# TMZZ22331/Robust-Speech-Emotion-Recognition-via-Dynamic-Asymmetric-Distillation-in-Noisy-Environments

Hardware: AMD Instinct MI355X
Metric: utterances/sec (DAD train step) batch=64 at 1/2/4/8 MI355X; loss parity (higher is better)
Workload: dtype fp16

## Files before the change

### robust-speech-emotion-recognition-via-dynamic-asymmetric-distillation-in-noisy-environments_amd/csrc/dad_abi.hip

```cpp
#include <string.h>

#include "dad_host.h"
#include "dad_timing.h"

constexpr int kMaxDevices = 64;

int device_cus(int* out) {
  static int cache[kMaxDevices];
  int dev = 0;
  DAD_TRY(hipGetDevice(&dev));
  if (dev < 0 || dev >= kMaxDevices) return DAD_E_ARG;
  if (!cache[dev]) DAD_TRY(hipDeviceGetAttribute(&cache[dev], hipDeviceAttributeMultiprocessorCount, dev));
  *out = cache[dev];
  return DAD_OK;
}

namespace {

inline DadStoreRows store_rows_of(const dad_batch* bt) { return DadStoreRows{bt->rowc, bt->lenc, bt->rown, bt->lenn}; }

DadPrepArgs prep_args(const dad_config* cfg, const dad_batch* bt, uint16_t* x16) {
  DadPrepArgs p;
  memset(&p, 0, sizeof(p));
  const Keys k = keys_of(cfg);
// ... 111 lines not shown
  memset(&pa, 0, sizeof(pa));
  pa.g = s.G; pa.warmup = cfg->warmup;
  pa.mc = bt->mc; pa.mn = bt->mn; pa.part_sum = s.ws.part_sum;
  pa.student = s.st->student; pa.teacher = s.st->teacher;
  if (s.explicit_rng()) { pa.keep1 = bt->keep1; pa.keep2 = bt->keep2; }
  pa.key_drop1 = s.k.drop1; pa.key_drop2 = s.k.drop2;
  pa.p_drop = cfg->p_drop; pa.drop_scale = cfg->drop_scale;
  pa.emb = s.st->emb; pa.vlen = s.ws.vlen; pa.logits = s.st->logits;
  pa.part_cnt = s.ws.part_cnt; pa.cnt_tot = s.ws.cnt_tot;
  pa.eflag = s.ws.eflag; pa.tail_terms = s.st->tail + DAD_T_ECDA_TERM;
  pa.range_flag = reinterpret_cast<uint32_t*>(s.st->tail + DAD_T_RANGE);
  if (cfg->ragged) { pa.lenc = bt->lenc; pa.lenn = bt->lenn; }
  if (!s.plan.pool_grid) pa.ready = s.ws.pool_ready;
  return pa;
}

DadTailArgs tail_args(const Step& s) {
  DadTailArgs ta;
  memset(&ta, 0, sizeof(ta));
  ta.cfg = *s.cfg; ta.yc = s.bt->yc; ta.logits = s.st->logits; ta.emb = s.st->emb; ta.student = s.st->student;
  if (s.explicit_rng()) { ta.keep1 = s.bt->keep1; ta.keep2 = s.bt->keep2; }
  ta.key_drop1 = s.k.drop1; ta.key_drop2 = s.k.drop2;
  ta.dacp = s.st->dacp; ta.tailf = s.st->tail; ta.ge = s.ws.ge; ta.ge_ecda = s.ws.ge_ecda; ta.grad = s.st->grad;
  ta.gzb = s.ws.gzb; ta.eflag = s.ws.eflag;
  return ta;
}

DadEcdaArgs ecda_args(const Step& s) {
  DadEcdaArgs ca;
  memset(&ca, 0, sizeof(ca));
  ca.cfg = *s.cfg; ca.yc = s.bt->yc; ca.emb = s.st->emb; ca.tailf = s.st->tail;
  ca.tail_terms = s.st->tail + DAD_T_ECDA_TERM; ca.ge = s.ws.ge_ecda; ca.scratch = s.ws.ecda; ca.eflag = s.ws.eflag;
  ca.sink = s.ws.gflat;
  return ca;
}

DadWgradArgs wgrad_args(const Step& s) {
  const dad_config* cfg = s.cfg;
  const dad_batch* bt = s.bt;
  DadWgradArgs wa;
  memset(&wa, 0, sizeof(wa));
  wa.g = s.G; wa.warmup = cfg->warmup;
  wa.mask_len = cfg->mask_len; wa.start_hi = cfg->start_hi;
  wa.xc = static_cast<const float*>(bt->xc); wa.xn = static_cast<const float*>(bt->xn);
  wa.src = store_rows_of(bt);
  if (s.explicit_rng()) { wa.ns = bt->ns; wa.u = bt->u; wa.start = bt->start; }
  wa.key_strong = s.k.strong; wa.key_feat = s.k.feat; wa.key_tstart = s.k.tstart;
  wa.strong_std = cfg->strong_std; wa.feat_p = cfg->feat_p;
  wa.bits = s.ws.bits; wa.ge = s.ws.ge; wa.vlen = s.ws.vlen; wa.xs16 = s.ws.set_of(cfg);
  wa.splits = s.plan.splits; wa.ntiles = s.plan.wgrad_tiles;
  wa.wpart = s.ws.wpart;
  return wa;
}

DadReduceArgs reduce_args(const Step& s) {
  const dad_config* cfg = s.cfg;
  DadReduceArgs ra;
  memset(&ra, 0, sizeof(ra));
  ra.g = s.G; ra.warmup = cfg->warmup;
  ra.want_norm = cfg->dp_world == 1;
  ra.w_kl = cfg->w_kl; ra.w_ecda = cfg->w_ecda;
  ra.w_scl = s.plan.scl_n ? cfg->w_scl : 0.0f;
  ra.ge_ecda = s.ws.ge_ecda;
  ra.gzb = s.ws.gzb; ra.eflag = s.ws.eflag; ra.student = s.st->student; ra.emb = s.st->emb;
  if (s.explicit_rng()) { ra.keep1 = s.bt->keep1; ra.keep2 = s.bt->keep2; }
  ra.key_drop1 = s.k.drop1; ra.key_drop2 = s.k.drop2; ra.p_drop = cfg->p_drop; ra.drop_scale = cfg->drop_scale;
// ... 314 lines not shown
```

### robust-speech-emotion-recognition-via-dynamic-asymmetric-distillation-in-noisy-environments_amd/csrc/dad_kernels.h

```cpp
#pragma once
#include "dad_common.h"

#define DAD_ENC_F32_THREADS 256
#define DAD_ENC_WS_THREADS 512
#define DAD_ENC_WS_MAXJ 256
#define DAD_POOL_THREADS 64
#define DAD_TAIL_THREADS 512
#define DAD_ECDA_THREADS 512
#define DAD_WGRAD_THREADS 256
#define WGD_DB 64
#define WGD_NDB (DAD_D / WGD_DB)
#define WGD_MAXU 64
#ifndef WGD_DEPTH
#define WGD_DEPTH 4
#endif
#define WGD_XP 96
#ifndef WGD_GROUPS
#define WGD_GROUPS 2
#endif
#define WGD_THREADS (256 * WGD_GROUPS)
#define WGD_XWG 4
#define DAD_REDUCE_THREADS 256
#define DAD_REDUCE_COLS 256
#define DAD_REDUCE_XBLK 16
// ... 54 lines not shown
  float weak_std, strong_std, feat_p;
  uint16_t* x16;
  __host__ __device__ int xc_type() const { return src_types & 0xff; }
  __host__ __device__ int xn_type() const { return (src_types >> 8) & 0xff; }
};


struct DadTailArgs {
  dad_config cfg;
  const int64_t* yc;
  const float* logits; const float* emb;
  const float* student;
  const uint8_t* keep1; const uint8_t* keep2;
  uint32_t key_drop1, key_drop2;
  float* dacp;
  float* tailf;
  float* ge;
  float* ge_ecda;
  float* gzb;
  uint32_t* eflag;
  float* grad;
};

struct DadEcdaArgs {
  dad_config cfg;
  const int64_t* yc;
  const float* emb;
  const float* tailf;
  float* tail_terms;
  float* ge;
  uint32_t* eflag;
  float* scratch;
  float* sink;
};

struct DadWgradArgs {
  DadGeom g;
  int warmup, splits, mask_len, start_hi;
  const float* xc; const float* xn;
  DadStoreRows src;
  const float* ns; const float* u; const int64_t* start;
  uint32_t key_strong, key_feat, key_tstart;
  float strong_std, feat_p;
  const uint32_t* bits; const float* ge; const float* vlen;
  const uint16_t* xs16;
  float* wpart;
  int ntiles;
};

struct DadReduceArgs {
  DadGeom g;
  int splits, warmup, want_norm;
  float w_kl, w_ecda;
  const float* wpart; const float* ge; const float* vlen; const float* cnt_tot;
  const float* ge_ecda;
  const float* gzb; const uint32_t* eflag;
  const float* student; const float* emb;
  const uint8_t* keep1; const uint8_t* keep2;
  uint32_t key_drop1, key_drop2;
  float p_drop, drop_scale;
  const float* tailf;
  float* grad; float* normpart;
  const uint32_t* pool_abort;
  float w_scl;
};

// ... 69 lines not shown
```

### robust-speech-emotion-recognition-via-dynamic-asymmetric-distillation-in-noisy-environments_amd/csrc/step_plan.h

```cpp
#pragma once
#include <stdlib.h>
#include <string.h>

#include <algorithm>
#include <vector>

#include "dad_kernels.h"
#include "scl.h"

inline int check_cfg(const dad_config* c) {
  if (!c) return DAD_E_ARG;
  if (c->B < 1 || c->B > DAD_MAX_BATCH || c->T < 1) return DAD_E_SHAPE;
  if (c->Bn < 0 || c->Bn > DAD_MAX_BATCH || c->Tn < 0) return DAD_E_SHAPE;
  if (!c->warmup && (c->Bn < 1 || c->Tn < 1)) return DAD_E_SHAPE;
  if (c->precision != DAD_PREC_FP32 && !dad_prec16(c->precision)) return DAD_E_ARG;
  if (c->rng_mode != DAD_RNG_EXPLICIT && c->rng_mode != DAD_RNG_COUNTER) return DAD_E_ARG;
  if (c->dp_world < 1) return DAD_E_ARG;
  if (c->ragged && !dad_prec16(c->precision)) return DAD_E_UNSUPPORTED;
  if (c->scl_on && !(scl_tau_ok(c->scl_tau) && c->w_scl >= -3.402823466e38f && c->w_scl <= 3.402823466e38f)) return DAD_E_ARG;
  return DAD_OK;
}

inline bool scl_in_step(const dad_config* c) { return c->scl_on && !c->warmup; }

// ... 5 lines not shown
inline bool store_dtype_ok(int t) { return t == DAD_STORE_F32 || t == DAD_STORE_F16 || t == DAD_STORE_BF16; }
inline int check_batch_dtypes(const dad_config* c, const dad_batch* b) {
  if (!store_dtype_ok(b->xc_dtype) || !store_dtype_ok(b->xn_dtype)) return DAD_E_ARG;
  if ((!b->rowc && b->xc_dtype != DAD_STORE_F32) || (!b->rown && b->xn_dtype != DAD_STORE_F32)) return DAD_E_ARG;
  if ((b->xc_dtype != DAD_STORE_F32 || b->xn_dtype != DAD_STORE_F32) && !dad_prec16(c->precision))
    return DAD_E_UNSUPPORTED;
  return DAD_OK;
}
inline int check_ragged_batch(const dad_config* c, const dad_batch* b) {
  if (!c->ragged) return DAD_OK;
  if (!b->rowc || !b->lenc) return DAD_E_ARG;
  if ((b->xn || !c->warmup) && (!b->rown || !b->lenn)) return DAD_E_ARG;
  return DAD_OK;
}
inline bool has_explicit_draws(const dad_batch* b) { return b->nw && b->ns && b->u && b->start; }

inline int splits_of(const dad_config* c) {
  const DadGeom g = geom_of(c);
  if (c->splits <= 0) return dad_auto_splits(g, c->precision, c->warmup);
  if (!dad_prec16(c->precision)) return c->splits;
  return std::max(c->splits, dad_wgd_min_splits(dad_wg_total(g, c->warmup)));
}

inline int max_splits_of(const dad_config* c) {
  const int s = splits_of(c);
  if (!c->warmup) return s;
  dad_config post = *c;
  post.warmup = 0;
  return std::max(s, splits_of(&post));
}

inline bool tail_w_on() {
  static const bool on = [] { const char* e = getenv("DAD_TAIL_W"); return !(e && strcmp(e, "0") == 0); }();
  return on;
}

inline int wp_max_range(const DadGeom& G, int Bn, int nt, int ns) {
  int worst = 0;
  for (int wg = 0; wg < nt + ns; ++wg) {
    bool t = false;
    int j0 = 0, j1 = 0;
    dad_wp_job_range(wg, nt, ns, G.Bc, G.Tc, G.ncc, Bn, G.Tn, G.ncn, Bn * G.ncn, t, j0, j1);
    worst = std::max(worst, j1 - j0);
  }
  return worst;
}
inline int wp_split(const DadGeom& G, int Bn, int cus, int& nt, int& ns) {
  struct Entry { int Bc, Tc, Bn, Tn, cus, rc, nt, ns; };
  static thread_local Entry last{-1, -1, -1, -1, -1, 0, 0, 0};
  if (!(last.Bc == G.Bc && last.Tc == G.Tc && last.Bn == Bn && last.Tn == G.Tn && last.cus == cus)) {
    Entry e{G.Bc, G.Tc, Bn, G.Tn, cus, 0, 0, 0};
    const int Js = Bn * G.ncn, Jc = G.Bc * G.ncc;
    const double ln = (double)Bn * ((G.Tn + 15) / 16), lc = (double)G.Bc * ((G.Tc + 15) / 16);
    if (Js == 0) {
      e.ns = std::min(cus, Jc);
    } else {
      e.nt = std::max(1, std::min(std::min(Js, cus - 1), (int)(cus * ln / (2.0 * ln + lc) + 0.5)));
      e.ns = std::min(cus - e.nt, Jc + Js);
    }
    while (e.rc == DAD_OK && wp_max_range(G, Bn, e.nt, e.ns) > DAD_ENC_WS_MAXJ) {
      if (e.nt > 0 && e.nt < Js) ++e.nt;
      if (e.ns < Jc + Js) ++e.ns;
      if (e.nt + e.ns > Js + Jc + 2) e.rc = DAD_E_SHAPE;
    }
    last = e;
  }
// ... 204 lines not shown
```

### robust-speech-emotion-recognition-via-dynamic-asymmetric-distillation-in-noisy-environments_amd/csrc/tail_w.hip

```cpp
#include "dad_prep.h"
#include "dad_probe.h"
#include "pool.h"
#include "tail_common.h"

#define ECDA_SLOTS 32
DAD_PROBE_BUFFER(ecda_stamps, DAD_C * ECDA_SLOTS + 16)
DAD_PROBE_BUFFER(prep_stamps, 256 * 8 * 2)
#define ECDA_STAMP(k) \
  if (threadIdx.x == 0) DAD_PROBE_SET(ecda_stamps, (blockIdx.x - 1) * ECDA_SLOTS + (k), DAD_PROBE_WALL())
#define ECDA_CYC(k)                                                                          \
  do {                                                                                       \
    __builtin_amdgcn_sched_barrier(0);                                                       \
    if (threadIdx.x == 0) DAD_PROBE_SET(ecda_stamps, (blockIdx.x - 1) * ECDA_SLOTS + (k), DAD_PROBE_CLK()); \
    __builtin_amdgcn_sched_barrier(0);                                                       \
  } while (0)
#define ECDA_STAMP_SIZES(c, n, ns) \
  do { DAD_PROBE_SET(ecda_stamps, (c) * ECDA_SLOTS + 10, (n)); DAD_PROBE_SET(ecda_stamps, (c) * ECDA_SLOTS + 11, (ns)); } while (0)
#define TAIL_STAMP(k) \
  if (threadIdx.x == 0) DAD_PROBE_SET(ecda_stamps, DAD_C * ECDA_SLOTS + (k), DAD_PROBE_WALL())
#define TAIL_CYCLES(k) \
  if (threadIdx.x == 0) DAD_PROBE_SET(ecda_stamps, DAD_C * ECDA_SLOTS + (k), DAD_PROBE_CLK())

#define TAIL_STAMP_W1(k) \
  if (threadIdx.x == 64 && blockIdx.x == 0) DAD_PROBE_SET(ecda_stamps, DAD_C * ECDA_SLOTS + (k), DAD_PROBE_WALL())

#define TW_MAXB 64
#define EW_ZP 260
#define EW_CP 68
#define EW_CPW 132
#define EW_GP 33

struct DacpBlockScratch {
  int rk[ECDA_THREADS / 64][TW_MAXB];
  float srt[ECDA_THREADS / 64][DAD_C][TW_MAXB];
};

struct DacpState {
  float tau[DAD_C], Q[DAD_C], anc[DAD_C];
};

template <int N>
__device__ __forceinline__ float dpp_seg_sum(float v) {
  static_assert(N == 4 || N == 8 || N == 16 || N == 32, "segment");
  v += dad_dpp_f<0x111>(v);
  v += dad_dpp_f<0x112>(v);
  if constexpr (N >= 8) v += dad_dpp_f<0x114>(v);
  if constexpr (N >= 16) v += dad_dpp_f<0x118>(v);
  if constexpr (N == 32) v += dad_dpp_f<0x142, 0xa>(v);
  return v;
}
__device__ __forceinline__ DacpState dacp_state_of(float dv) {
  DacpState d;
#pragma unroll
  for (int k = 0; k < DAD_C; ++k) {
    d.tau[k] = __int_as_float(__builtin_amdgcn_readlane(__float_as_int(dv), k));
    d.Q[k] = __int_as_float(__builtin_amdgcn_readlane(__float_as_int(dv), 4 + k));
    d.anc[k] = __int_as_float(__builtin_amdgcn_readlane(__float_as_int(dv), 16 + k));
  }
  return d;
}

__device__ __forceinline__ void dacp_block8(const dad_config& cfg, int Bn, float s, int p, const DacpState& D,
                                            DacpBlockScratch& W, float (&tau)[DAD_C], float (&wc)[DAD_C],
// ... 190 lines not shown
struct __attribute__((aligned(16))) EcdaW {
  union {
    float zc[(TW_MAXB + 1) * EW_ZP];
    float dbw[2 * TW_MAXB * EW_CPW];
  } a;
  union {
    DacpBlockScratch dw;
    float gp[10][32 * EW_GP];
  } b;
  union {
    float cp[ECDA_THREADS / 64][DAD_C][DAD_H];
    float dbn[TW_MAXB * EW_CP];
  } c;
  float cent[DAD_C][DAD_H];
  float nz[2 * TW_MAXB], wz[2 * TW_MAXB], rs[2 * TW_MAXB];
  int rowz[2 * TW_MAXB], mem[2 * TW_MAXB];
  int cnt[DAD_C];
  float pd[DAD_C][DAD_C];
  float msp[ECDA_THREADS / 64][DAD_H];
  double nsp[ECDA_THREADS / 64];
  double t3p[ECDA_THREADS / 64][3];
  float cmp[ECDA_THREADS / 64];
};

__device__ __forceinline__ int ew_pair(int ti, int tj, int nt) { return ti * nt - ti * (ti - 1) / 2 + (tj - ti); }
__device__ __forceinline__ void ew_pair_inv(int pr, int nt, int& ti, int& tj) {
  ti = 0;
  while (pr >= nt - ti) { pr -= nt - ti; ++ti; }
  tj = ti + pr;
}

#define EW_TP 40
static_assert(ECDA_NG * 32 * EW_TP <= sizeof(EcdaW::b) / sizeof(float), "ew_member_grads: a 32 x EW_TP tile per wave in S.b");
__device__ __forceinline__ int ew_nk64(int ncand_all) { return max((ncand_all + 7) >> 3, 5); }

template <int NP, int NK, class RG>
__device__ __forceinline__ void ew_member_grads(EcdaW& S, const float* db, int dp, int c, int ncs, int ncand_all,
                                                float mmd_scale, float comp_scale, float* ge_c, float* ge_s,
                                                float* sink, const RG& repg_at) {
  static_assert(NK >= 1 && NK <= NP / 8, "ew_member_grads: NK 8-candidate blocks of NP");
  const int tid = threadIdx.x, lane = tid & 63;
  const int g = __builtin_amdgcn_readfirstlane(tid >> 6);
  const int kh = lane >> 5, l32 = lane & 31;
  for (int item = g; item < (NP / 32) * (DAD_H / 32); item += ECDA_NG) {
    const int ti = item >> 3, tc = item & 7;
    const int d = 32 * tc + l32;
    const float* ra = &db[(32 * ti + l32) * dp + 4 * kh];
    f32x4 av[NK];
    float bv[NK][4];
#pragma unroll
    for (int q = 0; q < NK; ++q) {
      av[q] = *reinterpret_cast<const f32x4*>(ra + 8 * q);
#pragma unroll
      for (int e = 0; e < 4; ++e) bv[q][e] = S.a.zc[(8 * q + 4 * kh + e) * EW_ZP + d];
    }
    float zi[16], rsv[16];
#pragma unroll
    for (int r = 0; r < 16; ++r) {
      const int i = 32 * ti + dad_acc_row(r, kh);
      const int ic = i < ncand_all ? i : 0;
      zi[r] = S.a.zc[i * EW_ZP + d];
      rsv[r] = S.rs[ic];
    }
    const float mu = S.cent[c][d], rg = repg_at(d);
    f32x16 acc = f32x16{};
#pragma unroll
    for (int q = 0; q < NK; ++q)
#pragma unroll
      for (int e = 0; e < 4; ++e) acc = __builtin_amdgcn_mfma_f32_32x32x2f32(av[q][e], bv[q][e], acc, 0, 0, 0);
    ECDA_CYC(25);
    float* stg = &S.b.gp[0][0] + g * (32 * EW_TP);
#pragma unroll
    for (int r = 0; r < 16; ++r) {
      const int i = 32 * ti + dad_acc_row(r, kh);
      const bool noisy = i >= ncs;
      stg[dad_acc_row(r, kh) * EW_TP + l32] =
          mmd_scale * (2.0f * (rsv[r] * zi[r] - acc[r])) + (noisy ? comp_scale * (zi[r] - mu) + rg : 0.0f);
    }
    asm volatile("s_waitcnt lgkmcnt(0)" ::: "memory");
    ECDA_CYC(26);
    const int rl = lane >> 3, c4 = 4 * (lane & 7);
#pragma unroll
    for (int k = 0; k < 4; ++k) {
      const int row = rl + 8 * k, i = 32 * ti + row;
      const int ic = i < ncand_all ? i : 0;
      const bool mem = (i < ncand_all) & (S.mem[ic] != 0);
      const f32x4 v = *reinterpret_cast<const f32x4*>(stg + row * EW_TP + c4);
      float* dst = mem ? (i >= ncs ? ge_s : ge_c) + (size_t)S.rowz[ic] * DAD_H + 32 * tc + c4 : sink + 32 * tc + c4;
      *reinterpret_cast<f32x4*>(dst) = v;
    }
    asm volatile("s_waitcnt lgkmcnt(0)" ::: "memory");
    ECDA_CYC(27);
  }
}

template <bool WIDE>
__device__ __forceinline__ void ecda_class_w(const DadEcdaArgs& a, const int c, EcdaW& S, const WaveMask& M,
                                             const f32x4 (&ps)[ECDA_PRE_U], const int prd,
                                             const int ncls, const int nvalid, const int npairs, const bool gc,
                                             const bool rep_on, const float rep_coef, const float att_c, const int ncs,
                                             const int ncand_all, const double wsum_t) {
  const dad_config& cfg = a.cfg;
  const int B = cfg.B, Bn = cfg.Bn;
  const int tid = threadIdx.x, lane = tid & 63;
  const int g = __builtin_amdgcn_readfirstlane(tid >> 6);
  const int kh = lane >> 5, l32 = lane & 31;
  const float* emb_c = a.emb;
  const float* emb_s = a.emb + (size_t)(B + Bn) * DAD_H;
  const int npad = ncand_all <= 32 ? 32 : (ncand_all <= 64 ? 64 : 128);
  const int nt = npad / 32;
  const int npt = nt * (nt + 1) / 2;
  const int ks = npt == 1 ? 8 : (npt == 3 ? 2 : 1);
  float* db = WIDE ? S.a.dbw : S.c.dbn;
  const int dp = WIDE ? EW_CPW : EW_CP;
  const int cnc = S.cnt[c];
  const int nmem = ncs + cnc;
  auto rowp = [&](int i) -> const float* {
    if constexpr (WIDE) return (i < ncs ? emb_c : emb_s) + (size_t)S.rowz[i < ncand_all ? i : 0] * DAD_H;
    else return &S.a.zc[i * EW_ZP];
  };
  auto rowv = [&](int i, int col) -> float {
    if constexpr (WIDE) return i < ncand_all ? rowp(i)[col] : 0.0f;
    else return S.a.zc[i * EW_ZP + col];
  };
  if (gc) {
    f32x4 ms = f32x4{};
    double ns = 0.0;
    const f32x4 z0 = *reinterpret_cast<const f32x4*>(rowp(0) + 4 * lane);
    for (int r = g; r < ncand_all; r += ECDA_NG) {
      const f32x4 v = *reinterpret_cast<const f32x4*>(rowp(r) + 4 * lane);
      const float nr = dad_wave_sum(((v[0] * v[0] + v[1] * v[1]) + v[2] * v[2]) + v[3] * v[3]);
      if (lane == 0) S.nz[r] = nr;
      if (S.mem[r]) {
        const f32x4 d = v - z0;
        ms += d;
        ns += (double)dad_wave_sum(((d[0] * d[0] + d[1] * d[1]) + d[2] * d[2]) + d[3] * d[3]);
      }
    }
    *reinterpret_cast<f32x4*>(&S.msp[g][4 * lane]) = ms;
    if (lane == 0) S.nsp[g] = ns;
    for (int item = g; item < (npt == 3 ? 10 : npt * ks); item += ECDA_NG) {
      int pr, sl, nsl;
      if (npt == 3) {
        constexpr uint64_t kDeal = 0x2ull | (0x5ull << 4) | (0x8ull << 8) | (0x9ull << 12) | (0x3ull << 16) |
                                   (0x6ull << 20) | (0x0ull << 24) | (0x1ull << 28) | (0x4ull << 32) | (0x7ull << 36);
        const int v = (int)((kDeal >> (4 * item)) & 15u);
        pr = v >> 2;
        sl = v & 3;
        nsl = pr < 2 ? 4 : 2;
      } else {
        pr = item / ks;
        sl = item - pr * ks;
        nsl = ks;
      }
      const int slot = npt == 3 ? (pr < 2 ? 4 * pr : 8) + sl : item;
      int ti, tj;
      ew_pair_inv(pr, nt, ti, tj);
      const int kw = DAD_H / nsl, k0 = sl * kw;
      const int ia = 32 * ti + l32, ib = 32 * tj + l32;
      const float* ra = rowp(ia) + 4 * kh;
      const float* rb = rowp(ib) + 4 * kh;
      const bool za = WIDE && ia >= ncand_all, zb = WIDE && ib >= ncand_all;
      f32x16 acc = f32x16{};
      for (int k = k0; k < k0 + kw; k += 8) {
        f32x4 av = *reinterpret_cast<const f32x4*>(ra + k), bv = *reinterpret_cast<const f32x4*>(rb + k);
        if (za) av = f32x4{};
        if (zb) bv = f32x4{};
#pragma unroll
        for (int e = 0; e < 4; ++e) acc = __builtin_amdgcn_mfma_f32_32x32x2f32(av[e], bv[e], acc, 0, 0, 0);
      }
#pragma unroll
      for (int r = 0; r < 16; ++r) S.b.gp[slot][dad_acc_row(r, kh) * EW_GP + l32] = acc[r];
    }
  }
  for (int e = tid; e < DAD_C * DAD_H; e += ECDA_THREADS) {
    const int k = e >> 8, hh = e & (DAD_H - 1);
    float sk = 0.0f;
#pragma unroll
    for (int gg = 0; gg < ECDA_NG; ++gg) sk += S.c.cp[gg][k][hh];
    const int nk = S.cnt[k];
    S.cent[k][hh] = nk > 0 ? sk / (float)nk : 0.0f;
  }
  ECDA_STAMP(4);
  __syncthreads();
  ECDA_STAMP(5);
  ECDA_CYC(6);
  const int ept = npad * npad / ECDA_THREADS;
  const int tpr = npad / ept;
  const int ei = tid / tpr, ej0 = (tid - ei * tpr) * ept;
  {
    const int pair = tid / 32, t32 = tid & 31;
    float d = 0.0f;
    if (pair < DAD_C * DAD_C) {
      const int p = pair / DAD_C, q = pair % DAD_C;
      const int lo = p < q ? p : q, hi = p < q ? q : p;
      const int np = S.cnt[p];
      const int nq = S.cnt[q];
      if (p < ncls && q < ncls && np > 0 && nq > 0 && p != q) {
        const f32x4* a0 = reinterpret_cast<const f32x4*>(&S.cent[lo][t32 * (DAD_H / 32)]);
        const f32x4* a1 = reinterpret_cast<const f32x4*>(&S.cent[hi][t32 * (DAD_H / 32)]);
        const f32x4 x0 = a0[0], x1 = a0[1], y0 = a1[0], y1 = a1[1];
        const float v[8] = {x0[0] - y0[0], x0[1] - y0[1], x0[2] - y0[2], x0[3] - y0[3],
                            x1[0] - y1[0], x1[1] - y1[1], x1[2] - y1[2], x1[3] - y1[3]};
#pragma unroll
        for (int k = 0; k < 8; ++k) d += v[k] * v[k];
      }
    }
    d = dpp_seg_sum<32>(d);
    if (pair < DAD_C * DAD_C && t32 == 31) S.pd[pair / DAD_C][pair % DAD_C] = sqrtf(d);
  }
  ECDA_CYC(20);
  const float Wss = (float)ncs * (float)ncs + 1e-8f;
  const float Wtt = (float)(wsum_t * wsum_t) + 1e-8f;
  const float Wst = (float)((double)ncs * wsum_t) + 1e-8f;
  if (gc) {
    float cpart = 0.0f;
    const f32x4 mu = *reinterpret_cast<const f32x4*>(&S.cent[c][4 * lane]);
#pragma unroll
    for (int u = 0; u < ECDA_PRE_U; ++u) {
      const int b = g + ECDA_NG * u;
      const int pk = __builtin_amdgcn_readlane(prd, b < 64 ? b : 0);
      if (b < Bn && pk == c) {
        const f32x4 df = ps[u] - mu;
        cpart += ((df[0] * df[0] + df[1] * df[1]) + df[2] * df[2]) + df[3] * df[3];
      }
    }
    cpart = dad_wave_sum(cpart);
    f32x4 m = f32x4{};
#pragma unroll
    for (int gg = 0; gg < ECDA_NG; ++gg) m += *reinterpret_cast<const f32x4*>(&S.msp[gg][4 * lane]);
    const double msq = dad_wave_sum_d(((double)m[0] * m[0] + (double)m[1] * m[1]) + ((double)m[2] * m[2] + (double)m[3] * m[3]));
    double nsq = 0.0;
#pragma unroll
    for (int gg = 0; gg < ECDA_NG; ++gg) nsq += S.nsp[gg];
    const double bws = fmax(2.0 * (double)nmem * nsq - 2.0 * msq, 0.0);
    float bw = nmem > 1 ? (float)(bws / (double)(nmem * nmem - nmem)) : 1.0f;
    bw = bw / 4.0f;
    float ibw[5];
#pragma unroll
    for (int mm = 0; mm < 5; ++mm) ibw[mm] = 1.0f / (bw * (float)(1 << mm) + 1e-8f);
    ECDA_CYC(21);
    double t3[3] = {0.0, 0.0, 0.0};
    float rsp = 0.0f;
    const int ic = ei < ncand_all ? ei : 0;
    const bool mi = (ei < ncand_all) & (S.mem[ic] != 0);
    const float wi = S.wz[ic];
    const bool si = ei < ncs;
    const float css = 2.0f / Wss, ctt = 2.0f / Wtt, cst = -2.0f / Wst;
    auto coef = [&](const int j) {
      const int i = ei;
      const int lo = i < j ? i : j, hi = i < j ? j : i;
      const int pr = ew_pair(lo >> 5, hi >> 5, nt);
      float gsum = 0.0f;
      const int sb = npt == 3 ? (pr < 2 ? 4 * pr : 8) : pr * ks, sn = npt == 3 ? (pr < 2 ? 4 : 2) : ks;
      for (int s2 = 0; s2 < sn; ++s2) gsum += S.b.gp[sb + s2][(lo & 31) * EW_GP + (hi & 31)];
      const bool ok = (i < ncand_all) & (j < ncand_all) & (i != j);
      const float d = ok ? fmaxf((S.nz[lo] + S.nz[hi]) - 2.0f * gsum, 0.0f) : 0.0f;
      const int jc = j < ncand_all ? j : 0;
      const bool on = mi & (j < ncand_all) & (S.mem[jc] != 0);
      const float wj = S.wz[jc];
      float K = 0.0f, dK = 0.0f;
#pragma unroll
      for (int mm = 0; mm < 5; ++mm) {
        const float ex = __expf(-d * ibw[mm]);
        K += ex;
        dK -= ex * ibw[mm];
      }
      const bool sj = j < ncs;
      const bool ss = on & si & sj, tt = on & !si & !sj, st = on & si & !sj, ts = on & !si & sj;
      const float ww = wi * wj;
      t3[0] += ss ? (double)K : 0.0;
      t3[1] += tt ? (double)K * ww : 0.0;
      t3[2] += st ? (double)K * wj : 0.0;
      const float vss = css * dK, vtt = (ctt * ww) * dK, vst = (cst * wj) * dK, vts = (cst * wi) * dK;
      float v = ss ? vss : (tt ? vtt : (st ? vst : (ts ? vts : 0.0f)));
      v = i == j ? 0.0f : v;
      rsp += v;
      return v;
    };
    if (!WIDE && npad == 64) {
      const int jt = ej0 / ept, kz = 8 * ew_nk64(ncand_all);
      float v8[8];
#pragma unroll
      for (int e = 0; e < 8; ++e) {
        const int j = jt + 8 * e;
        v8[e] = (j < kz && ei < ncand_all) ? coef(j) : 0.0f;
      }
#pragma unroll
      for (int e = 0; e < 8; ++e)
        if (jt + 8 * e < kz) db[ei * dp + jt + 8 * e] = v8[e];
    } else {
      for (int e = 0; e < ept; ++e) db[ei * dp + ej0 + e] = coef(ej0 + e);
    }
    ECDA_CYC(22);
    rsp = tpr == 16 ? dpp_seg_sum<16>(rsp) : (tpr == 8 ? dpp_seg_sum<8>(rsp) : dpp_seg_sum<4>(rsp));
    if ((tid & (tpr - 1)) == tpr - 1) S.rs[ei] = rsp;
#pragma unroll
    for (int k = 0; k < 3; ++k) t3[k] = dad_wave_sum_d(t3[k]);
    if (lane == 0) { S.t3p[g][0] = t3[0]; S.t3p[g][1] = t3[1]; S.t3p[g][2] = t3[2]; S.cmp[g] = cpart; }
    ECDA_CYC(23);
  }
  __syncthreads();
  ECDA_STAMP(7);
  const float wscale = cfg.w_ecda;
  float pd[DAD_C][DAD_C];
#pragma unroll
  for (int p = 0; p < DAD_C; ++p)
#pragma unroll
    for (int q = 0; q < DAD_C; ++q) pd[p][q] = S.pd[p][q];
  float rep = 0.0f;
  if (nvalid > 1) {
    float sp = 0.0f;
#pragma unroll
    for (int p = 0; p < DAD_C; ++p)
#pragma unroll
      for (int q = p + 1; q < DAD_C; ++q) {
        const int np = S.cnt[p];
        const int nq = S.cnt[q];
        if (q < ncls && np > 0 && nq > 0) sp += pd[p][q];
      }
    rep = -sp / (float)npairs;
  }
  float rq[DAD_C];
// ... 7 lines not shown
  auto repg_at = [&](int d) -> float {
    if (!rep_on) return 0.0f;
    const float cc0 = S.cent[c][d];
    float gsum = 0.0f;
#pragma unroll
    for (int q = 0; q < DAD_C; ++q) gsum += rq[q] != 0.0f ? (cc0 - S.cent[q][d]) * rq[q] : 0.0f;
    return rk * gsum;
  };
  float* ge_c = a.ge;
  float* ge_s = a.ge + (size_t)B * DAD_H;
  if (gc) {
    double t3[3] = {0.0, 0.0, 0.0};
#pragma unroll
    for (int gg = 0; gg < ECDA_NG; ++gg) {
      t3[0] += S.t3p[gg][0];
      t3[1] += S.t3p[gg][1];
      t3[2] += S.t3p[gg][2];
    }
    const float mmd = (float)t3[0] / Wss + (float)t3[1] / Wtt - 2.0f * ((float)t3[2] / Wst);
    float csum = 0.0f;
#pragma unroll
    for (int gg = 0; gg < ECDA_NG; ++gg) csum += S.cmp[gg];
    const float comp = csum / (float)cnc;
    if (tid == 0) {
      a.tail_terms[c] = att_c * (mmd + cfg.ecda_gamma * comp + cfg.ecda_delta * rep);
      a.tail_terms[DAD_T_ECDA_GATE - DAD_T_ECDA_TERM + c] = 1.0f;
    }
    ECDA_CYC(24);
    const float mmd_scale = wscale * att_c;
    const float comp_scale = wscale * att_c * cfg.ecda_gamma * (2.0f / (float)cnc);
    if constexpr (!WIDE) {
      if (npad == 32) {
        ew_member_grads<32, 4>(S, db, dp, c, ncs, ncand_all, mmd_scale, comp_scale, ge_c, ge_s, a.sink, repg_at);
      } else {
        const int nk = ew_nk64(ncand_all);
        if (nk <= 5) ew_member_grads<64, 5>(S, db, dp, c, ncs, ncand_all, mmd_scale, comp_scale, ge_c, ge_s, a.sink, repg_at);
        else if (nk == 6) ew_member_grads<64, 6>(S, db, dp, c, ncs, ncand_all, mmd_scale, comp_scale, ge_c, ge_s, a.sink, repg_at);
        else if (nk == 7) ew_member_grads<64, 7>(S, db, dp, c, ncs, ncand_all, mmd_scale, comp_scale, ge_c, ge_s, a.sink, repg_at);
        else ew_member_grads<64, 8>(S, db, dp, c, ncs, ncand_all, mmd_scale, comp_scale, ge_c, ge_s, a.sink, repg_at);
      }
    }
    for (int item = g; WIDE && item < nt * (DAD_H / 32); item += ECDA_NG) {
      const int ti = item >> 3, tc = item & 7;
      const int d = 32 * tc + l32;
      f32x16 acc = f32x16{};
      const float* ra = &db[(32 * ti + l32) * dp + 4 * kh];
      for (int k = 0; k < npad; k += 8) {
        const f32x4 av = *reinterpret_cast<const f32x4*>(ra + k);
        float bv[4];
#pragma unroll
        for (int e = 0; e < 4; ++e) bv[e] = rowv(k + 4 * kh + e, d);
#pragma unroll
        for (int e = 0; e < 4; ++e) acc = __builtin_amdgcn_mfma_f32_32x32x2f32(av[e], bv[e], acc, 0, 0, 0);
      }
      const float mu = S.cent[c][d], rg = repg_at(d);
#pragma unroll
      for (int r = 0; r < 16; ++r) {
        const int i = 32 * ti + dad_acc_row(r, kh);
        const int ic = i < ncand_all ? i : 0;
        const bool ok = (i < ncand_all) & (S.mem[ic] != 0);
        const float zi = rowv(i, d);
        const bool noisy = i >= ncs;
        const float gv = mmd_scale * (2.0f * (S.rs[ic] * zi - acc[r])) + (noisy ? comp_scale * (zi - mu) + rg : 0.0f);
        float* dst = ok ? (noisy ? ge_s : ge_c) + (size_t)S.rowz[ic] * DAD_H + d : a.sink + d;
        *dst = gv;
      }
    }
  } else {
// ... 82 lines not shown
    if (gated[k]) rep_coef += att[k] * cfg.ecda_delta;
  }
  const int cnc = c == 0 ? cn[0] : (c == 1 ? cn[1] : (c == 2 ? cn[2] : cn[3]));
  const int ccc = c == 0 ? cc[0] : (c == 1 ? cc[1] : (c == 2 ? cc[2] : cc[3]));
  const bool gc = c == 0 ? gated[0] : (c == 1 ? gated[1] : (c == 2 ? gated[2] : gated[3]));
  const float att_c = sel4(att, c);
  const bool rep_on = nvalid > 1 && cnc > 0 && rep_coef != 0.0f;
  ECDA_CYC(13);
  if (!gc && !rep_on) return;
  const bool ccand = gc && y == c;
  const bool ncand = lane < Bn && M.p == c && M.m;
  const uint64_t bc = __ballot(ccand), bn = __ballot(ncand);
  const int ncs = gc ? ccc : 0;
  const int ncand_all = ncs + (int)__popcll(bn);
  const bool wide = ncand_all > TW_MAXB;
  const uint64_t below = (1ull << lane) - 1ull;
  const int posc = (int)__popcll(bc & below);
  const int posn = ncs + (int)__popcll(bn & below);
  int npos[2 * ECDA_PRE_U];
#pragma unroll
  for (int u = 0; u < ECDA_PRE_U; ++u) {
    const int b = g + ECDA_NG * u;
    const bool okc = gc & (b < ncl);
    const bool okn = (b < Bn) & (((bn >> b) & 1ull) != 0);
    npos[2 * u] = __builtin_amdgcn_readfirstlane(okc ? b : -1);
    npos[2 * u + 1] = __builtin_amdgcn_readfirstlane(okn ? __builtin_amdgcn_readlane(posn, b) : -1);
    if (!wide & okc) *reinterpret_cast<f32x4*>(&S.a.zc[npos[2 * u] * EW_ZP + 4 * lane]) = pc[u];
    if (!wide & okn) *reinterpret_cast<f32x4*>(&S.a.zc[npos[2 * u + 1] * EW_ZP + 4 * lane]) = ps[u];
  }
  ECDA_CYC(14);
  ECDA_STAMP(12);
  ECDA_CYC(15);
  if (!wide) {
    const int npad = ncand_all <= 32 ? 32 : 64;
    for (int r = ncand_all + g; r < npad; r += ECDA_NG) *reinterpret_cast<f32x4*>(&S.a.zc[r * EW_ZP + 4 * lane]) = f32x4{};
  }
  if (g == 0) {
    if (lane < DAD_C) S.cnt[lane] = sel4i(cn, lane);
    if (ccand) { S.rowz[posc] = lane; S.wz[posc] = 1.0f; S.mem[posc] = 1; }
    if (ncand) { S.rowz[posn] = lane; S.wz[posn] = M.s; S.mem[posn] = 1; }
  }
  ECDA_CYC(16);
  {
    f32x4 cs0 = f32x4{}, cs1 = f32x4{}, cs2 = f32x4{}, cs3 = f32x4{};
#pragma unroll
    for (int u = 0; u < ECDA_PRE_U; ++u) {
      const int b = g + ECDA_NG * u;
      const int pk = __builtin_amdgcn_readfirstlane(b < Bn ? __builtin_amdgcn_readlane(prd, b < 64 ? b : 0) : -1);
      cs0 += ps[u] * (pk == 0 ? 1.0f : 0.0f);
      cs1 += ps[u] * (pk == 1 ? 1.0f : 0.0f);
      cs2 += ps[u] * (pk == 2 ? 1.0f : 0.0f);
      cs3 += ps[u] * (pk == 3 ? 1.0f : 0.0f);
    }
    *reinterpret_cast<f32x4*>(&S.c.cp[g][0][4 * lane]) = cs0;
    *reinterpret_cast<f32x4*>(&S.c.cp[g][1][4 * lane]) = cs1;
    *reinterpret_cast<f32x4*>(&S.c.cp[g][2][4 * lane]) = cs2;
    *reinterpret_cast<f32x4*>(&S.c.cp[g][3][4 * lane]) = cs3;
  }
  ECDA_CYC(17);
  const double wsum_t = dad_wave_sum_d(ncand ? (double)M.s : 0.0);
  (void)cc;
  ECDA_CYC(18);
  ECDA_STAMP(2);
  __syncthreads();
  ECDA_STAMP(3);
  if (wide)
    ecda_class_w<true>(a, c, S, M, ps, prd, ncls, nvalid, npairs, gc, rep_on, rep_coef, att_c, ncs, ncand_all, wsum_t);
  else
    ecda_class_w<false>(a, c, S, M, ps, prd, ncls, nvalid, npairs, gc, rep_on, rep_coef, att_c, ncs, ncand_all, wsum_t);
}

#if defined(DAD_TAIL_W_RG)
#define TAIL_W_KERNEL dad_tail_ecda_w_rg
#define DAD_TAIL_W_S16 1
#elif defined(DAD_TAIL_W_S16)
#define TAIL_W_KERNEL dad_tail_ecda_w_s16
#define DAD_TAIL_W_RG 0
#else
#define TAIL_W_KERNEL dad_tail_ecda_w
#define DAD_TAIL_W_S16 0
#define DAD_TAIL_W_RG 0
#endif
__global__ __launch_bounds__(TAIL_THREADS) void TAIL_W_KERNEL(DadTailArgs ta, DadEcdaArgs ca, DadPrepArgs pa,
                                                                DadPoolArgs pl) {
  DAD_GUARD_BLOCK(TAIL_THREADS);
  __shared__ union UW {
    TailW t;
    EcdaW e;
  } u;
  const int nitems = pl.ready ? pl.g.Bc + 2 * pl.g.Bn : 0;
  if ((int)blockIdx.x > DAD_C) {
    constexpr int kWaves = TAIL_THREADS / 64;
    const int w = __builtin_amdgcn_readfirstlane((int)threadIdx.x >> 6);
    const int nx = (int)gridDim.x - 1 - DAD_C, xb = (int)blockIdx.x - 1 - DAD_C;
    for (int i = xb + nx * w; i < nitems; i += nx * kWaves) {
      pool_item<true, DAD_TAIL_W_RG>(pl, i, (int)threadIdx.x & 63);
      pool_publish(pl.ready, (int)threadIdx.x & 63);
    }
    if (!pa.x16) return;
#ifdef DAD_PROBE_STAMPS
// ... 16 lines not shown
```

Baseline: 660,900.

## Add 48-row padded tiling for ECDA Gram and member grads with 33-48 candidates

Adds a new narrow-path specialization of the ECDA class kernel for classes with 33 to 48 candidates. These are padded to 48 rows and use 16x16x4 MFMA tiles, both for the Gram matrix (split into 3x3 16-row blocks across the 8 waves) and for the member-gradient GEMM, instead of padding to 64 and using 32x32 tiles. The aim is to cut the wasted MFMA work and LDS traffic spent on padded rows. The path is on by default and can be turned off with an environment variable. It adds a third template instantiation and new LDS indexing, which raises register pressure and the risk of indexing mistakes.

```diff
diff --git a/robust-speech-emotion-recognition-via-dynamic-asymmetric-distillation-in-noisy-environments_amd/csrc/dad_abi.hip b/robust-speech-emotion-recognition-via-dynamic-asymmetric-distillation-in-noisy-environments_amd/csrc/dad_abi.hip
--- a/robust-speech-emotion-recognition-via-dynamic-asymmetric-distillation-in-noisy-environments_amd/csrc/dad_abi.hip
+++ b/robust-speech-emotion-recognition-via-dynamic-asymmetric-distillation-in-noisy-environments_amd/csrc/dad_abi.hip
@@ -167,6 +167,7 @@
   ca.cfg = *s.cfg; ca.yc = s.bt->yc; ca.emb = s.st->emb; ca.tailf = s.st->tail;
   ca.tail_terms = s.st->tail + DAD_T_ECDA_TERM; ca.ge = s.ws.ge_ecda; ca.scratch = s.ws.ecda; ca.eflag = s.ws.eflag;
   ca.sink = s.ws.gflat;
+  ca.tile48 = ecda_tile48_on() ? 1 : 0;
   return ca;
 }
 
diff --git a/robust-speech-emotion-recognition-via-dynamic-asymmetric-distillation-in-noisy-environments_amd/csrc/dad_kernels.h b/robust-speech-emotion-recognition-via-dynamic-asymmetric-distillation-in-noisy-environments_amd/csrc/dad_kernels.h
--- a/robust-speech-emotion-recognition-via-dynamic-asymmetric-distillation-in-noisy-environments_amd/csrc/dad_kernels.h
+++ b/robust-speech-emotion-recognition-via-dynamic-asymmetric-distillation-in-noisy-environments_amd/csrc/dad_kernels.h
@@ -110,6 +110,7 @@
   uint32_t* eflag;
   float* scratch;
   float* sink;
+  int tile48;
 };
 
 struct DadWgradArgs {
diff --git a/robust-speech-emotion-recognition-via-dynamic-asymmetric-distillation-in-noisy-environments_amd/csrc/step_plan.h b/robust-speech-emotion-recognition-via-dynamic-asymmetric-distillation-in-noisy-environments_amd/csrc/step_plan.h
--- a/robust-speech-emotion-recognition-via-dynamic-asymmetric-distillation-in-noisy-environments_amd/csrc/step_plan.h
+++ b/robust-speech-emotion-recognition-via-dynamic-asymmetric-distillation-in-noisy-environments_amd/csrc/step_plan.h
@@ -61,6 +61,11 @@
 
 inline bool tail_w_on() {
   static const bool on = [] { const char* e = getenv("DAD_TAIL_W"); return !(e && strcmp(e, "0") == 0); }();
+  return on;
+}
+
+inline bool ecda_tile48_on() {
+  static const bool on = [] { const char* e = getenv("DAD_ECDA_TILE48"); return !(e && strcmp(e, "0") == 0); }();
   return on;
 }
 
diff --git a/robust-speech-emotion-recognition-via-dynamic-asymmetric-distillation-in-noisy-environments_amd/csrc/tail_w.hip b/robust-speech-emotion-recognition-via-dynamic-asymmetric-distillation-in-noisy-environments_amd/csrc/tail_w.hip
--- a/robust-speech-emotion-recognition-via-dynamic-asymmetric-distillation-in-noisy-environments_amd/csrc/tail_w.hip
+++ b/robust-speech-emotion-recognition-via-dynamic-asymmetric-distillation-in-noisy-environments_amd/csrc/tail_w.hip
@@ -29,6 +29,12 @@
 #define EW_CP 68
 #define EW_CPW 132
 #define EW_GP 33
+#define EW_GP16 17
+#define EW_G16 (16 * EW_GP16)
+
+__device__ __forceinline__ int ew_npad(int ncand_all, int tile48) {
+  return ncand_all <= 32 ? 32 : ((ncand_all <= 48) & (tile48 != 0) ? 48 : 64);
+}
 
 struct DacpBlockScratch {
   int rk[ECDA_THREADS / 64][TW_MAXB];
@@ -285,7 +291,7 @@
 
 #define EW_TP 40
 static_assert(ECDA_NG * 32 * EW_TP <= sizeof(EcdaW::b) / sizeof(float), "ew_member_grads: a 32 x EW_TP tile per wave in S.b");
-__device__ __forceinline__ int ew_nk64(int ncand_all) { return max((ncand_all + 7) >> 3, 5); }
+__device__ __forceinline__ int ew_nk(int ncand_all) { return max((ncand_all + 7) >> 3, 5); }
 
 template <int NP, int NK, class RG>
 __device__ __forceinline__ void ew_member_grads(EcdaW& S, const float* db, int dp, int c, int ncs, int ncand_all,
@@ -347,7 +353,93 @@
   }
 }
 
-template <bool WIDE>
+#define EW_TP16 36
+template <int NK, class RG>
+__device__ __forceinline__ void ew_member_grads48(EcdaW& S, const float* db, int dp, int c, int ncs, int ncand_all,
+                                                  float mmd_scale, float comp_scale, float* ge_c, float* ge_s,
+                                                  float* sink, const RG& repg_at) {
+  static_assert(NK == 5 || NK == 6, "ew_member_grads48: 33..48 candidates, 5 or 6 8-candidate blocks");
+  constexpr int NQ = NK == 6 ? 3 : 2;
+  const int tid = threadIdx.x, lane = tid & 63;
+  const int g = __builtin_amdgcn_readfirstlane(tid >> 6);
+  const int kq = lane >> 4, l16 = lane & 15;
+  constexpr int NS = 2 * NK;
+  static_assert(DAD_H / 32 == ECDA_NG, "ew_member_grads48: one 32-unit column tile per wave");
+  static_assert(2 * 16 * EW_TP16 <= 32 * EW_TP, "ew_member_grads48: two 16 x EW_TP16 tiles in the wave's tile of S.b");
+  float* stg = &S.b.gp[0][0] + g * (32 * EW_TP);
+  const int d0 = 32 * g + l16;
+  auto kk = [&](int s) { return s < 4 * NQ ? 16 * (s >> 2) + 4 * kq + (s & 3) : 32 + 2 * kq + (s - 4 * NQ); };
+  float bv[NS][2];
+#pragma unroll
+  for (int s = 0; s < NS; ++s) {
+    bv[s][0] = S.a.zc[kk(s) * EW_ZP + d0];
+    bv[s][1] = S.a.zc[kk(s) * EW_ZP + d0 + 16];
+  }
+  float av[3][NS], zi[3][4][2], rsv[3][4];
+#pragma unroll
+  for (int ti = 0; ti < 3; ++ti) {
+    const float* ra = &db[(16 * ti + l16) * dp];
+#pragma unroll
+    for (int q = 0; q < NQ; ++q) {
+      const f32x4 t = *reinterpret_cast<const f32x4*>(ra + 16 * q + 4 * kq);
+#pragma unroll
+      for (int e = 0; e < 4; ++e) av[ti][4 * q + e] = t[e];
+    }
+    if constexpr (NK == 5) {
+      const f32x2 t = *reinterpret_cast<const f32x2*>(ra + 32 + 2 * kq);
+      av[ti][8] = t[0];
+      av[ti][9] = t[1];
+    }
+#pragma unroll
+    for (int r = 0; r < 4; ++r) {
+      const int i = 16 * ti + 4 * kq + r;
+      const int ic = i < ncand_all ? i : 0;
+      zi[ti][r][0] = S.a.zc[i * EW_ZP + d0];
+      zi[ti][r][1] = S.a.zc[i * EW_ZP + d0 + 16];
+      rsv[ti][r] = S.rs[ic];
+    }
+  }
+  const float mu[2] = {S.cent[c][d0], S.cent[c][d0 + 16]};
+  const float rg[2] = {repg_at(d0), repg_at(d0 + 16)};
+  f32x4 acc[3][2];
+#pragma unroll
+  for (int ti = 0; ti < 3; ++ti) acc[ti][0] = acc[ti][1] = f32x4{};
+#pragma unroll
+  for (int s = 0; s < NS; ++s)
+#pragma unroll
+    for (int ti = 0; ti < 3; ++ti) {
+      acc[ti][0] = __builtin_amdgcn_mfma_f32_16x16x4f32(av[ti][s], bv[s][0], acc[ti][0], 0, 0, 0);
+      acc[ti][1] = __builtin_amdgcn_mfma_f32_16x16x4f32(av[ti][s], bv[s][1], acc[ti][1], 0, 0, 0);
+    }
+  ECDA_CYC(25);
+  const int rl = lane >> 3, c4 = 4 * (lane & 7);
+#pragma unroll
+  for (int ti = 0; ti < 3; ++ti) {
+    float* tile = stg + (ti & 1) * (16 * EW_TP16);
+#pragma unroll
+    for (int r = 0; r < 4; ++r) {
+      const int i = 16 * ti + 4 * kq + r;
+      const bool noisy = i >= ncs;
+      float* o = tile + (4 * kq + r) * EW_TP16 + l16;
+      o[0] = mmd_scale * (2.0f * (rsv[ti][r] * zi[ti][r][0] - acc[ti][0][r])) + (noisy ? comp_scale * (zi[ti][r][0] - mu[0]) + rg[0] : 0.0f);
+      o[16] = mmd_scale * (2.0f * (rsv[ti][r] * zi[ti][r][1] - acc[ti][1][r])) + (noisy ? comp_scale * (zi[ti][r][1] - mu[1]) + rg[1] : 0.0f);
+    }
+    asm volatile("s_waitcnt lgkmcnt(0)" ::: "memory");
+    if (ti == 2) ECDA_CYC(26);
+#pragma unroll
+    for (int k = 0; k < 2; ++k) {
+      const int row = rl + 8 * k, i = 16 * ti + row;
+      const int ic = i < ncand_all ? i : 0;
+      const bool mem = (i < ncand_all) & (S.mem[ic] != 0);
+      const f32x4 v = *reinterpret_cast<const f32x4*>(tile + row * EW_TP16 + c4);
+      float* dst = mem ? (i >= ncs ? ge_s : ge_c) + (size_t)S.rowz[ic] * DAD_H + 32 * g + c4 : sink + 32 * g + c4;
+      *reinterpret_cast<f32x4*>(dst) = v;
+    }
+  }
+  ECDA_CYC(27);
+}
+
+template <bool WIDE, bool T48 = false>
 __device__ __forceinline__ void ecda_class_w(const DadEcdaArgs& a, const int c, EcdaW& S, const WaveMask& M,
                                              const f32x4 (&ps)[ECDA_PRE_U], const int prd,
                                              const int ncls, const int nvalid, const int npairs, const bool gc,
@@ -360,8 +452,10 @@
   const int kh = lane >> 5, l32 = lane & 31;
   const float* emb_c = a.emb;
   const float* emb_s = a.emb + (size_t)(B + Bn) * DAD_H;
-  const int npad = ncand_all <= 32 ? 32 : (ncand_all <= 64 ? 64 : 128);
-  const int nt = npad / 32;
+  static_assert(!(WIDE && T48), "ecda_class_w: the 48-row tiling is a narrow one");
+  constexpr bool t48 = T48;
+  const int npad = T48 ? 48 : (ncand_all <= 32 ? 32 : (ncand_all <= 64 ? 64 : 128));
+  const int nt = T48 ? 2 : npad / 32;
   const int npt = nt * (nt + 1) / 2;
   const int ks = npt == 1 ? 8 : (npt == 3 ? 2 : 1);
   float* db = WIDE ? S.a.dbw : S.c.dbn;
@@ -392,7 +486,38 @@
     }
     *reinterpret_cast<f32x4*>(&S.msp[g][4 * lane]) = ms;
     if (lane == 0) S.nsp[g] = ns;
-    for (int item = g; item < (npt == 3 ? 10 : npt * ks); item += ECDA_NG) {
+    if constexpr (T48) {
+      static_assert(24 * EW_G16 <= sizeof(EcdaW::b) / sizeof(float), "48-row tiling: 24 Gram partial tiles in S.b");
+      const int kq = lane >> 4, l16 = lane & 15;
+      const int sl = g & 3;
+      const bool odd = g >= 4;
+      const float* r0 = &S.a.zc[l16 * EW_ZP + 64 * sl + 4 * kq];
+      const float* r1 = r0 + 16 * EW_ZP;
+      const float* r2 = r0 + 32 * EW_ZP;
+      f32x4 c0 = f32x4{}, c1 = f32x4{}, c2 = f32x4{};
+#pragma unroll
+      for (int k = 0; k < 64; k += 16) {
+        const f32x4 x0 = *reinterpret_cast<const f32x4*>(r0 + k);
+        const f32x4 x1 = *reinterpret_cast<const f32x4*>(r1 + k);
+        const f32x4 x2 = *reinterpret_cast<const f32x4*>(r2 + k);
+        const f32x4 a1 = odd ? x1 : x0, b0 = odd ? x1 : x0;
+        const f32x4 a2 = odd ? x2 : x1, b1 = odd ? x1 : x2;
+#pragma unroll
+        for (int e = 0; e < 4; ++e) {
+          c0 = __builtin_amdgcn_mfma_f32_16x16x4f32(x0[e], b0[e], c0, 0, 0, 0);
+          c1 = __builtin_amdgcn_mfma_f32_16x16x4f32(a1[e], b1[e], c1, 0, 0, 0);
+          c2 = __builtin_amdgcn_mfma_f32_16x16x4f32(a2[e], x2[e], c2, 0, 0, 0);
+        }
+      }
+      float* gq = &S.b.gp[0][0] + (4 * (int)odd + sl) * EW_G16 + 4 * kq * EW_GP16 + l16;
+#pragma unroll
+      for (int r = 0; r < 4; ++r) {
+        gq[r * EW_GP16] = c0[r];
+        gq[8 * EW_G16 + r * EW_GP16] = c1[r];
+        gq[16 * EW_G16 + r * EW_GP16] = c2[r];
+      }
+    }
+    for (int item = g; !t48 && item < (npt == 3 ? 10 : npt * ks); item += ECDA_NG) {
       int pr, sl, nsl;
       if (npt == 3) {
         constexpr uint64_t kDeal = 0x2ull | (0x5ull << 4) | (0x8ull << 8) | (0x9ull << 12) | (0x3ull << 16) |
@@ -438,8 +563,9 @@
   __syncthreads();
   ECDA_STAMP(5);
   ECDA_CYC(6);
-  const int ept = npad * npad / ECDA_THREADS;
-  const int tpr = npad / ept;
+  const int npo = t48 ? 64 : npad;
+  const int ept = npo * npo / ECDA_THREADS;
+  const int tpr = npo / ept;
   const int ei = tid / tpr, ej0 = (tid - ei * tpr) * ept;
   {
     const int pair = tid / 32, t32 = tid & 31;
@@ -503,10 +629,16 @@
     auto coef = [&](const int j) {
       const int i = ei;
       const int lo = i < j ? i : j, hi = i < j ? j : i;
-      const int pr = ew_pair(lo >> 5, hi >> 5, nt);
       float gsum = 0.0f;
-      const int sb = npt == 3 ? (pr < 2 ? 4 * pr : 8) : pr * ks, sn = npt == 3 ? (pr < 2 ? 4 : 2) : ks;
-      for (int s2 = 0; s2 < sn; ++s2) gsum += S.b.gp[sb + s2][(lo & 31) * EW_GP + (hi & 31)];
+      if constexpr (T48) {
+        const float* gq = &S.b.gp[0][0] + 4 * ew_pair(lo >> 4, hi >> 4, 3) * EW_G16 + (lo & 15) * EW_GP16 + (hi & 15);
+#pragma unroll
+        for (int s2 = 0; s2 < 4; ++s2) gsum += gq[s2 * EW_G16];
+      } else {
+        const int pr = ew_pair(lo >> 5, hi >> 5, nt);
+        const int sb = npt == 3 ? (pr < 2 ? 4 * pr : 8) : pr * ks, sn = npt == 3 ? (pr < 2 ? 4 : 2) : ks;
+        for (int s2 = 0; s2 < sn; ++s2) gsum += S.b.gp[sb + s2][(lo & 31) * EW_GP + (hi & 31)];
+      }
       const bool ok = (i < ncand_all) & (j < ncand_all) & (i != j);
       const float d = ok ? fmaxf((S.nz[lo] + S.nz[hi]) - 2.0f * gsum, 0.0f) : 0.0f;
       const int jc = j < ncand_all ? j : 0;
@@ -532,7 +664,7 @@
       return v;
     };
     if (!WIDE && npad == 64) {
-      const int jt = ej0 / ept, kz = 8 * ew_nk64(ncand_all);
+      const int jt = ej0 / ept, kz = 8 * ew_nk(ncand_all);
       float v8[8];
 #pragma unroll
       for (int e = 0; e < 8; ++e) {
@@ -542,6 +674,17 @@
 #pragma unroll
       for (int e = 0; e < 8; ++e)
         if (jt + 8 * e < kz) db[ei * dp + jt + 8 * e] = v8[e];
+    } else if (t48) {
+      const int jt = ej0 / ept, kz = 8 * ew_nk(ncand_all);
+      float v6[6];
+#pragma unroll
+      for (int e = 0; e < 6; ++e) {
+        const int j = jt + 8 * e;
+        v6[e] = (j < kz && ei < ncand_all) ? coef(j) : 0.0f;
+      }
+#pragma unroll
+      for (int e = 0; e < 6; ++e)
+        if (jt + 8 * e < kz) db[ei * dp + jt + 8 * e] = v6[e];
     } else {
       for (int e = 0; e < ept; ++e) db[ei * dp + ej0 + e] = coef(ej0 + e);
     }
@@ -615,8 +758,11 @@
     if constexpr (!WIDE) {
       if (npad == 32) {
         ew_member_grads<32, 4>(S, db, dp, c, ncs, ncand_all, mmd_scale, comp_scale, ge_c, ge_s, a.sink, repg_at);
+      } else if (t48) {
+        if (ew_nk(ncand_all) <= 5) ew_member_grads48<5>(S, db, dp, c, ncs, ncand_all, mmd_scale, comp_scale, ge_c, ge_s, a.sink, repg_at);
+        else ew_member_grads48<6>(S, db, dp, c, ncs, ncand_all, mmd_scale, comp_scale, ge_c, ge_s, a.sink, repg_at);
       } else {
-        const int nk = ew_nk64(ncand_all);
+        const int nk = ew_nk(ncand_all);
         if (nk <= 5) ew_member_grads<64, 5>(S, db, dp, c, ncs, ncand_all, mmd_scale, comp_scale, ge_c, ge_s, a.sink, repg_at);
         else if (nk == 6) ew_member_grads<64, 6>(S, db, dp, c, ncs, ncand_all, mmd_scale, comp_scale, ge_c, ge_s, a.sink, repg_at);
         else if (nk == 7) ew_member_grads<64, 7>(S, db, dp, c, ncs, ncand_all, mmd_scale, comp_scale, ge_c, ge_s, a.sink, repg_at);
@@ -765,7 +911,7 @@
   ECDA_STAMP(12);
   ECDA_CYC(15);
   if (!wide) {
-    const int npad = ncand_all <= 32 ? 32 : 64;
+    const int npad = ew_npad(ncand_all, a.tile48);
     for (int r = ncand_all + g; r < npad; r += ECDA_NG) *reinterpret_cast<f32x4*>(&S.a.zc[r * EW_ZP + 4 * lane]) = f32x4{};
   }
   if (g == 0) {
@@ -799,6 +945,8 @@
   ECDA_STAMP(3);
   if (wide)
     ecda_class_w<true>(a, c, S, M, ps, prd, ncls, nvalid, npairs, gc, rep_on, rep_coef, att_c, ncs, ncand_all, wsum_t);
+  else if (ew_npad(ncand_all, a.tile48) == 48)
+    ecda_class_w<false, true>(a, c, S, M, ps, prd, ncls, nvalid, npairs, gc, rep_on, rep_coef, att_c, ncs, ncand_all, wsum_t);
   else
     ecda_class_w<false>(a, c, S, M, ps, prd, ncls, nvalid, npairs, gc, rep_on, rep_coef, att_c, ncs, ncand_all, wsum_t);
 }
```

Result: no change. 658,600 (-0.4%).
